# gereonsuch/gr-FDC

Hardware: AMD Instinct MI355X
Metric: complex Msamples/s in, 64k-FFT/256-ch overlap-save; achieved HBM GB/s vs peak (higher is better)
Workload: dtype f32

## Files before the change

gr-fdc_amd/csrc/fdc_block256.hip:

```cpp
#include "fdc_blockcommon.hpp"
#include "fdc_iq.hpp"

namespace fdc {

extern __shared__ __attribute__((aligned(16))) unsigned char fdc_smem_blk[];

typedef unsigned long long u8v __attribute__((ext_vector_type(8)));

template <int P, bool OFF, bool FWD, bool R4, class TO>
constexpr bool kBlkSpread = !OFF && !FWD && !(P == 8 && (R4 || !std::is_same<TO, float2>::value));

template <int P>
struct BlkGeom {
    static_assert(P == 2 || P == 4 || P == 8, "passes of 32 columns: N = 16384, 32768 or 65536");
    static constexpr int kN1 = 32 * P;
    static constexpr int kN = 256 * kN1;
    static constexpr int kJT = P == 8 ? 4 : 8;
    static constexpr int kJB = P == 8 ? 2 : P == 4 ? 4 : 8;
    static constexpr int kLd = P == 2 ? 32 * P + 2 : 32 * P + 6;
    static constexpr int kTripBytes = 16 * kJT * kLd * 8;
    static constexpr int kOffCt = kTripBytes > kStripsEnd ? kTripBytes : kStripsEnd;
    static constexpr int kOffWrow = P == 8 ? 136960 : kOffCt + 32 * P * 8;
    static constexpr bool kSplit = P > 2;
    static constexpr int kOffLT = kOffWrow + 16 * 18 * 8;
    static constexpr int kOffUR = kOffLT + 64 * 18 * 8;
    static constexpr int kOffB = kOffLT, kOffSA = kOffB + 32 * 18 * 8;
    static constexpr int kOffSoff = kSplit ? kOffUR + kN1 * 4 * 8 : kOffSA + 16 * P * 18 * 8;
    static constexpr int kOffCbl = kOffSoff + kN1 * 4;
    static constexpr int kLds = kOffCbl + (kSplit ? (P + 8) * 16 * 8 : 0);
    static constexpr int kOffWrowF = kLds;
    static constexpr int kLdsOff = kOffWrowF + 16 * 18 * 8;
    static_assert(kLdsOff <= 160 * 1024 && kLds <= 160 * 1024, "LDS budget");
    static_assert(kOffCt >= kStripsEnd && kOffCt + 32 * P * 8 <= kOffWrow, "stage-2 trip buffer and twiddles below the tables, tables above the strips");
    static_assert((16 * (kJB - 1) * kLd + 32 * (P - 1)) * 8 < 65536, "ds offsets of a base register");
};


template <int P, bool NT, bool OFF, bool FWD, bool R4 = false, bool HALF = false, class TI = float2, class TO = float2, bool SPREAD = false>
__global__ FDC_PLAIN_DS __launch_bounds__(512, (P == 2 && !OFF && !R4 && !FWD) ? 4 : 2) void k_blk256(const TI *__restrict__ in, size_t in_stride, TO *__restrict__ out,
                                                const float2 *__restrict__ tw256, const float2 *__restrict__ twq,
                                                const float2 *__restrict__ cbt, const float *__restrict__ shn,
                                                const long long *__restrict__ slot_off, long long out_base,
                                                long long nb_call, unsigned out_bytes, int nb, int hints,
                                                unsigned long long *__restrict__ dbg , int roff, long long first_block,
                                                float2 *__restrict__ fwd_scratch, const unsigned *__restrict__ keep,
                                                typename IqTail<TI, TO>::type gpow )
{
    typedef BlkGeom<P> GM;
    constexpr bool kIq = !std::is_same<TI, float2>::value, kOq = !std::is_same<TO, float2>::value;
    static_assert(!SPREAD || kBlkSpread<P, OFF, FWD, R4, TO>, "no spread form of this one");
    static_assert(!kIq || !FWD, "integer input: the channelizer forms (the forward transform takes widened input)");
    static_assert(!kOq || !FWD, "integer output: the channelizer forms");
    constexpr unsigned kEs = (unsigned)sizeof(TI);
    constexpr unsigned kOs = (unsigned)sizeof(TO);
    [[maybe_unused]] const float iq_scale = iq_tail_scale(gpow);
    [[maybe_unused]] const float oq_scale = oq_tail_scale(gpow);
    static_assert(!HALF || (!OFF && !FWD), "the half-slot form is a variant of the on-grid channelizer");
    constexpr int kN1 = GM::kN1, kLd = GM::kLd, kJT = GM::kJT, kJB = GM::kJB;
    float2 *scr = reinterpret_cast<float2 *>(fdc_smem_blk);
    float2 *wrow = reinterpret_cast<float2 *>(fdc_smem_blk + GM::kOffWrow);
    constexpr bool kSplit = GM::kSplit;
    float2 *LT = reinterpret_cast<float2 *>(fdc_smem_blk + GM::kOffLT);
    float2 *UR = reinterpret_cast<float2 *>(fdc_smem_blk + GM::kOffUR);
    float2 *CBL = reinterpret_cast<float2 *>(fdc_smem_blk + GM::kOffCbl);
    float2 *Bt = reinterpret_cast<float2 *>(fdc_smem_blk + GM::kOffB);
    float2 *SA = reinterpret_cast<float2 *>(fdc_smem_blk + GM::kOffSA);
    unsigned *soff = reinterpret_cast<unsigned *>(fdc_smem_blk + GM::kOffSoff);
    float2 *ctab = reinterpret_cast<float2 *>(fdc_smem_blk + GM::kOffCt);
    const int tid = threadIdx.x;
    const int w = tid >> 6, lane = tid & 63, col = lane & 3, b = lane >> 2, c5 = 4 * w + col;
    unsigned mqs[4] = {~0u, ~0u, ~0u, ~0u};
    if (FWD && keep) {
        const int wu = __builtin_amdgcn_readfirstlane(w) % P;
#pragma unroll
        for (int q = 0; q < 4; q++) mqs[q] = keep[wu * 4 + q];
    }

    const int grid = gridDim.x, first = xcd_first_block();
    if (first >= nb) return;

    constexpr unsigned inbytes = (unsigned)GM::kN * kEs;
    constexpr unsigned kRowGrp = (unsigned)kN1 * 16u * kEs;
    const unsigned voff = (unsigned)(b * kN1 + c5) * kEs;
    [[maybe_unused]] auto ld_in = [&](__amdgpu_buffer_rsrc_t r, unsigned soff, auto aux) __attribute__((always_inline)) -> cf {
        constexpr int kAux = decltype(aux)::value;
        if constexpr (sizeof(TI) == 4) return mk(__uint_as_float(__builtin_amdgcn_raw_buffer_load_b32(r, voff, soff, kAux)), 0.f);
        else return mk(__uint_as_float((unsigned)__builtin_amdgcn_raw_buffer_load_b16(r, voff, soff, kAux)), 0.f);
    };
    [[maybe_unused]] const __amdgpu_buffer_rsrc_t rcb = make_rsrc(cbt, (unsigned)kN1 * 16u * 8u);
    [[maybe_unused]] const unsigned voffc = (unsigned)(c5 * 16 + b) * 8u;
    cf LA[16], LB[16], cbA = mk(1.f, 0.f), cbB = cbA;
    {
        const __amdgpu_buffer_rsrc_t rin = make_rsrc(in + (size_t)first * in_stride, inbytes);
#pragma unroll
        for (int a = 0; a < 16; a++) {
            if constexpr (kIq) LA[a] = ld_in(rin, (unsigned)a * kRowGrp, std::integral_constant<int, 0>{});
            else LA[a] = bld2(rin, voff, (unsigned)a * kRowGrp);
        }
        if constexpr (!kSplit) cbA = bld2(rcb, voffc, 0);
    }
    float2 *wrowF = OFF ? reinterpret_cast<float2 *>(fdc_smem_blk + GM::kOffWrowF) : wrow;
    const int r16 = roff & 15;
    for (int i = tid; i < 256; i += 512) {
        const int ip = (i >> 4) * 18 + (((i & 15) - 1) & 15);
        wrow[ip] = tw256[((i >> 4) * (i & 15)) & 255];
        if (OFF)
            wrowF[ip] = tw256[((i >> 4) * ((((i & 15) - r16) & 15) + roff)) & 255];
    }
    for (int i = tid; i < kN1; i += 512) {
        const long long o = slot_off[i];
        soff[(i % P) * 32 + ((i / P) & 1) * 16 + rev16((i / P) >> 1)] = o >= 0 ? (unsigned)((o * nb_call + out_base) * kOs) : 0xFFFFFFFFu;
    }
    for (int i = tid; i < 32 * P; i += 512) ctab[i] = tw256[((i / P) * (i % P) * (8 / P)) & 255];
    if constexpr (kSplit) {
        for (int i = tid; i < 1024; i += 512) {
            const int ln = i >> 4, q = i & 15, qt = HALF ? q ^ 8 : q;
            const float2 t = twq[(ln & 3) * 16 + qt];
            const float s = shn[(ln >> 2) + 16 * qt];
            const float2 e = make_float2(t.x * s, t.y * s), c = cbt[(ln & 3) * 16 + (ln >> 2)];
            LT[ln * 18 + q] = make_float2(e.x * c.x - e.y * c.y, e.x * c.y + e.y * c.x);
        }
        for (int i = tid; i < kN1 * 4; i += 512) UR[i] = twq[(i >> 4) * 64 + (HALF ? (i & 15) ^ 8 : i & 15)];
        if (tid < (P + 8) * 16)
            CBL[tid] = cbt[(tid < P * 16 ? (tid >> 4) * 512 : ((tid >> 4) - P) * 64) + (tid & 15)];
    } else {
        Bt[(tid >> 4) * 18 + (tid & 15)] = twq[HALF ? tid ^ 8 : tid];
        for (int i = tid; i < 256 * P; i += 512) {
            const int ps = i >> 8, bb = (i >> 4) & 15, q = i & 15, qt = HALF ? q ^ 8 : q;
            const float2 t = twq[(size_t)(32 * ps) * 16 + qt];
            const float s = shn[bb + 16 * qt];
            SA[(ps * 16 + bb) * 18 + q] = make_float2(t.x * s, t.y * s);
        }
    }
    __syncthreads();

    float2 *const scrw = scr + w * kStripPts + lane;
    const float2 *const scrr = scr + w * kStripPts + col + 68 * b;
    const float2 *const wr = wrow + b * 18;
    const float2 *const wrf = wrowF + b * 18;
    const float2 *const tr0 = kSplit ? UR + w * 16 : Bt + c5 * 18;
    const float2 *const tr1 = kSplit ? LT + lane * 18 : SA + b * 18;
    const float2 *const cblr = CBL + b;
    const __amdgpu_buffer_rsrc_t rout = make_rsrc(out, out_bytes);
    constexpr bool kScr = FWD || R4;
    const __amdgpu_buffer_rsrc_t rscr = make_rsrc(kScr ? fwd_scratch + (size_t)blockIdx.x * 32768 : fwd_scratch, kScr ? 32768u * 8u : 0u);


    for (int m = first; m < nb; m += grid) {
        const int mnext = m + grid < nb ? m + grid : m;
        const float sgn = (OFF && !R4 && (roff & 1) && ((first_block + m) & 1)) ? -1.0f : 1.0f;
        cf phs = mk(1.f, 0.f);
        if constexpr (OFF && R4) {
            const int pc = (int)((((first_block + m) & 3) * (roff & 3)) & 3);
            phs = mk(pc == 0 ? 1.f : pc == 2 ? -1.f : 0.f, pc == 1 ? 1.f : pc == 3 ? -1.f : 0.f);
        }
        typedef unsigned long long gvec __attribute__((ext_vector_type(P)));
        gvec G[8];
#define FDC_GGET(j, ps) unpack_cf(G[j][ps])
#define FDC_GPUT(j, ps, val) G[j][ps] = pack_cf(val)
        auto one_pass = [&](const int ps, cf (&cur)[16], const cf cbc, cf (&L)[16], cf &cbn) __attribute__((always_inline)) {
            const cf cbl = kSplit ? cmul(ld2(&cblr[16 * ps]), ld2(&cblr[16 * (P + w)])) : cbc;
            const cf cb = (OFF && R4) ? cmul(cbl, phs) : OFF ? cbl * sgn : cbl;
            const int pn = ps < P - 1 ? ps + 1 : 0;
            const int mb = ps < P - 1 ? m : mnext;
            const __amdgpu_buffer_rsrc_t rin = make_rsrc(in + (size_t)mb * in_stride + 32 * pn, inbytes);
            if constexpr (!SPREAD) {
                if constexpr (kIq) {
                    if (hints & 2) {
#pragma unroll
                        for (int a = 0; a < 16; a++) L[a] = ld_in(rin, (unsigned)a * kRowGrp, std::integral_constant<int, 2>{});
                    } else {
#pragma unroll
                        for (int a = 0; a < 16; a++) L[a] = ld_in(rin, (unsigned)a * kRowGrp, std::integral_constant<int, 0>{});
                    }
                } else if (hints & 2) {
#pragma unroll
                    for (int a = 0; a < 16; a++) L[a] = bld2_nt(rin, voff, (unsigned)a * kRowGrp);
                } else {
#pragma unroll
                    for (int a = 0; a < 16; a++) L[a] = bld2(rin, voff, (unsigned)a * kRowGrp);
                }
                if constexpr (!kSplit) cbn = bld2(rcb, voffc, (unsigned)pn * 4096u);
            }
            auto ld_rows = [&](auto group) __attribute__((always_inline)) {
                constexpr int g = decltype(group)::value;
                if constexpr (SPREAD) {
                    __builtin_amdgcn_sched_barrier(0);
#pragma unroll
                    for (int a = 4 * g; a < 4 * g + 4; a++) {
                        if constexpr (kIq) L[a] = ld_in(rin, (unsigned)a * kRowGrp, std::integral_constant<int, 0>{});
                        else L[a] = bld2(rin, voff, (unsigned)a * kRowGrp);
                    }
                    if constexpr (!kSplit && g == 3) cbn = bld2(rcb, voffc, (unsigned)pn * 4096u);
                }
            };
            const float2 *const r0 = tr0 + (kSplit ? 128 * ps : 0), *const r1 = tr1 + (kSplit ? 0 : 288 * ps);
            if constexpr (kIq) {
#pragma unroll
                for (int a = 0; a < 16; a++) cur[a] = iq_widen_bits(TI{}, __float_as_uint(cur[a].x), iq_scale);
            }
            dft16<false>(cur);
            ld_rows(std::integral_constant<int, 0>{});
            cf tw[16];
            ld_row_sh<OFF>(tw, wrf);
            if constexpr (OFF) {
#pragma unroll
                for (int p = 0; p < 16; p++) st2(&scrw[68 * ((p - r16) & 15)], cmul(cur[rev16(p)], tw[p]));
            } else {
                st2(&scrw[0], cur[rev16(0)]);
#pragma unroll
                for (int p = 1; p < 16; p++) st2(&scrw[68 * p], cmul(cur[rev16(p)], tw[p]));
            }
            __builtin_amdgcn_wave_barrier();
            cf v[16];
            strip_get(v, scrr);
            if constexpr (FWD) {
                dft16<false>(v);
#pragma unroll
                for (int i = 0; i < 8; i++) {
                    const float4 t0 = ld4(&r0[2 * i]), t1 = ld4(&r1[2 * i]);
                    const cf y0 = cmul(cmul(cmul(v[rev16(2 * i)], mk(t0.x, t0.y)), mk(t1.x, t1.y)), cb);
                    const cf y1 = cmul(cmul(cmul(v[rev16(2 * i + 1)], mk(t0.z, t0.w)), mk(t1.z, t1.w)), cb);
                    if (i < 4) { FDC_GPUT(2 * i, ps, y0); FDC_GPUT(2 * i + 1, ps, y1); }
                    else {
                        bst2(rscr, (unsigned)tid * 8u + (unsigned)(2 * i - 8) * 4096u, (unsigned)ps * 32768u, y0);
                        bst2(rscr, (unsigned)tid * 8u + (unsigned)(2 * i - 7) * 4096u, (unsigned)ps * 32768u, y1);
                    }
                }
            } else {
                dft16<false>(v);
                ld_rows(std::integral_constant<int, 1>{});
                cf u[16];
                {
#pragma unroll
                    for (int i = 0; i < 8; i++) {
                        const float4 t0 = ld4(&r0[2 * i]), t1 = ld4(&r1[2 * i]);
                        u[HALF ? 2 * i : (2 * i) ^ 8] = cmul(cmul(v[rev16(2 * i)], mk(t0.x, t0.y)), mk(t1.x, t1.y));
                        u[HALF ? 2 * i + 1 : (2 * i + 1) ^ 8] = cmul(cmul(v[rev16(2 * i + 1)], mk(t0.z, t0.w)), mk(t1.z, t1.w));
                    }
                }
                dft16<true>(u);
                ld_rows(std::integral_constant<int, 2>{});
                ld_row_sh<false>(tw, wr);
                u[rev16(0)] = cmul(u[rev16(0)], cb);
#pragma unroll
                for (int p = 1; p < 16; p++) u[rev16(p)] = cmul(cmulc(u[rev16(p)], tw[p]), cb);
                strip_trip(u, scrw, scrr);
                ld_rows(std::integral_constant<int, 3>{});
                dft16<true>(u);
                if constexpr (SPREAD) __builtin_amdgcn_sched_barrier(0);
#pragma unroll
                for (int j = 0; j < 8; j++) FDC_GPUT(j, ps, u[rev16(8 + j)]);
                if constexpr (SPREAD) __builtin_amdgcn_sched_barrier(0);
                if constexpr (R4) {
#pragma unroll
                    for (int j = 0; j < 4; j++) bst2(rscr, (unsigned)tid * 8u + (unsigned)j * 4096u, (unsigned)ps * 16384u, u[rev16(4 + j)]);
                }
            }
        };
        if constexpr (OFF && P == 8) {
#pragma nounroll
            for (int ps = 0; ps < P; ps++) {
                cf cur[16];
#pragma unroll
                for (int a = 0; a < 16; a++) cur[a] = LA[a];
                one_pass(ps, cur, cbA, LA, cbA);
            }
        } else {
#pragma nounroll
            for (int pp = 0; pp < P; pp += 2) {
                one_pass(pp, LA, cbA, LB, cbB);
                one_pass(pp + 1, LB, cbB, LA, cbA);
            }
        }
        auto stage2 = [&](auto get, const int rowbase, auto njc) __attribute__((always_inline)) {
            constexpr int kNJ = decltype(njc)::value;
            constexpr int kNTrip = (kNJ + kJT - 1) / kJT;
            __syncthreads();
            int t2 = tid;
            asm volatile("" : "+v"(t2));
            const int lane2 = t2 & 63, w2 = __builtin_amdgcn_readfirstlane(t2 >> 6), b_2 = lane2 >> 2, c5_2 = 4 * w2 + (lane2 & 3);
            const int klo2 = w2 % P, rh2 = w2 / P;
            float2 *const gw0 = scr + b_2 * kLd + c5_2;
            int rowjb = 16 * kJB * kLd;
            asm volatile("" : "+v"(rowjb));
            float2 *const gw1 = gw0 + rowjb;
            const float2 *const gr = scr + (64 * rh2 + lane2) * kLd + 32 * klo2;
            const uint4 *const sow = reinterpret_cast<const uint4 *>(soff + 32 * klo2);
#pragma unroll
            for (int tr = 0; tr < kNTrip; tr++) {
                const int ja = kNJ - kJT * tr < kJT ? kNJ - kJT * tr : kJT;
                cf ct[P];
                {
                    const float2 *ctr = reinterpret_cast<const float2 *>(fdc_smem_blk + GM::kOffCt) + c5_2 * P;
#pragma unroll
                    for (int i = 0; i < P / 2; i++) {
                        const float4 t = ld4(&ctr[2 * i]);
                        ct[2 * i] = mk(t.x, t.y); ct[2 * i + 1] = mk(t.z, t.w);
                    }
                }
                cf src[kJT][P];
#pragma unroll
                for (int jj = 0; jj < kJT; jj++)
#pragma unroll
                    for (int ps = 0; ps < P; ps++) if (jj < ja) src[jj][ps] = get(kJT * tr + jj, ps);
#pragma unroll
                for (int jj = 0; jj < kJT; jj++) {
                    if (jj >= ja) continue;
                    cf a[P];
#pragma unroll
                    for (int ps = 0; ps < P; ps++) a[ps] = src[jj][ps];
                    pass_dft<P>(a);
                    float2 *const gw = (jj < kJB ? gw0 : gw1) + (jj % kJB) * 16 * kLd;
                    st2(&gw[0], a[0]);
#pragma unroll
                    for (int k = 1; k < P; k++) st2(&gw[32 * k], cmul(a[pass_idx<P>(k)], ct[k]));
                }
                __builtin_amdgcn_sched_barrier(0);
                __syncthreads();
                const bool reads = P == 8 || 4 * rh2 < ja;
                cf v[32];
                if (reads) {
#pragma unroll
                    for (int i = 0; i < 16; i++) {
                        const float4 t = ld4(&gr[2 * i]);
                        v[2 * i] = mk(t.x, t.y); v[2 * i + 1] = mk(t.z, t.w);
                    }
                }
                __syncthreads();
                __builtin_amdgcn_sched_barrier(0);
                if (reads) {
                    dft32<false>(v);
                    const int trow0 = 16 * kJT * tr + 64 * rh2, trow = trow0 + lane2;
                    const unsigned rb = (unsigned)(m * (FWD ? GM::kN : (R4 ? 192 : 128)) + rowbase + trow) * kOs;
                    unsigned mq = FWD ? mqs[((rowbase + trow0) >> 6) & 3] : ~0u;
                    if constexpr (FWD) asm volatile("" : "+s"(mq));
#pragma unroll
                    for (int q = 0; q < 8; q++) {
                        const uint4 t = sow[q];
                        const unsigned so[4] = {t.x, t.y, t.z, t.w};
#pragma unroll
                        for (int e = 0; e < 4; e++) {
                            const unsigned o = FWD ? (so[e] | (((mq >> (4 * q + e)) & 1u) - 1u)) : so[e];
                            if constexpr (kOq) {
                                const unsigned u = oq_bits(TO{}, v[4 * q + e], oq_scale);
                                if constexpr (kOs == 4) __builtin_amdgcn_raw_buffer_store_b32(u, rout, (o == 0xFFFFFFFFu ? 0xFFFFFFF0u : o + rb), 0, NT ? 2 : 0);
                                else __builtin_amdgcn_raw_buffer_store_b16((unsigned short)u, rout, (o == 0xFFFFFFFFu ? 0xFFFFFFF0u : o + rb), 0, NT ? 2 : 0);
                            } else
                                bst2t<NT>(rout, (o == 0xFFFFFFFFu ? 0xFFFFFFF0u : o + rb), v[4 * q + e]);
                        }
                    }
                    if constexpr (FWD) {
                        if (gpow) {
                            float t16[16];
#pragma unroll
                            for (int i = 0; i < 16; i++) {
                                const float s0 = __builtin_fmaf(v[i].y, v[i].y, v[i].x * v[i].x);
                                const float s1 = __builtin_fmaf(v[i + 16].y, v[i + 16].y, v[i + 16].x * v[i + 16].x);
                                asm("s_nop 1\n\tv_add_f32_dpp %0, %1, %1 row_ror:8 row_mask:0xf bank_mask:0x3\n\t"
                                    "v_add_f32_dpp %0, %2, %2 row_ror:8 row_mask:0xf bank_mask:0xc" : "=&v"(t16[i]) : "v"(s0), "v"(s1));
                            }
                            float t8[8];
#pragma unroll
                            for (int i = 0; i < 8; i++)
                                asm("s_nop 1\n\tv_add_f32_dpp %0, %1, %1 row_shl:4 row_mask:0xf bank_mask:0x5\n\t"
                                    "v_add_f32_dpp %0, %2, %2 row_shr:4 row_mask:0xf bank_mask:0xa" : "=&v"(t8[i]) : "v"(t16[i]), "v"(t16[i + 8]));
                            const bool b1 = (lane2 & 2) != 0, b0 = (lane2 & 1) != 0;
                            float t4[4], t2[2];
#pragma unroll
                            for (int i = 0; i < 4; i++) {
                                const float keepv = b1 ? t8[i + 4] : t8[i], send = b1 ? t8[i] : t8[i + 4];
                                t4[i] = keepv + __builtin_bit_cast(float, __builtin_amdgcn_update_dpp(0, __builtin_bit_cast(int, send), 0x4E , 0xF, 0xF, false));
                            }
#pragma unroll
                            for (int i = 0; i < 2; i++) {
                                const float keepv = b0 ? t4[i + 2] : t4[i], send = b0 ? t4[i] : t4[i + 2];
                                t2[i] = keepv + __builtin_bit_cast(float, __builtin_amdgcn_update_dpp(0, __builtin_bit_cast(int, send), 0xB1 , 0xF, 0xF, false));
                            }
                            const int i16 = lane2 & 15, rho = lane2 >> 4, gsrc = 2 * (i16 & 1);
                            const int a0 = (16 * gsrc + 4 * rho + (i16 >> 2)) * 4, a1 = a0 + 64;
                            const int z0 = __builtin_bit_cast(int, t2[0]), z1 = __builtin_bit_cast(int, t2[1]);
                            const int f0a = __builtin_amdgcn_ds_bpermute(a0, z0), f0b = __builtin_amdgcn_ds_bpermute(a0, z1);
                            const int f1a = __builtin_amdgcn_ds_bpermute(a1, z0), f1b = __builtin_amdgcn_ds_bpermute(a1, z1);
                            const bool odd = (i16 & 2) != 0;
                            float2 pr;
                            pr.x = __builtin_bit_cast(float, odd ? f0b : f0a);
                            pr.y = __builtin_bit_cast(float, odd ? f1b : f1a);
                            const int reg = 8 * rho + (i16 >> 1), slot = klo2 + P * ((reg >> 4) + 2 * (4 * (reg & 3) + ((reg & 15) >> 2)));
                            *reinterpret_cast<float2 *>(gpow + (size_t)m * (GM::kN / 16) + 16 * slot + (rowbase + trow0) / 16 + gsrc) = pr;
                        }
                    }
                }
                __builtin_amdgcn_sched_barrier(0);
            }
        };
        stage2([&](int j, int ps) { return FDC_GGET(j, ps); }, R4 ? 64 : 0, std::integral_constant<int, 8>{});
        if constexpr (FWD) {
            asm volatile("s_waitcnt vmcnt(0)" ::: "memory");
            stage2([&](int j, int ps) { return bld2_sc1(rscr, (unsigned)tid * 8u + (unsigned)(j * 4096 + ps * 32768), 0u); }, 128,
                   std::integral_constant<int, 8>{});
        }
        if constexpr (R4) {
            asm volatile("s_waitcnt vmcnt(0)" ::: "memory");
            stage2([&](int j, int ps) { return bld2_sc1(rscr, (unsigned)tid * 8u + (unsigned)(j * 4096 + ps * 16384), 0u); }, 0,
                   std::integral_constant<int, 4>{});
        }
    }
}

template <int P, bool NT, bool OFF, bool FWD, bool R4, bool HALF, class TI, class TO, bool SPREAD>
constexpr bool blk256_form()
{
    constexpr bool kIq = !std::is_same<TI, float2>::value, kOq = !std::is_same<TO, float2>::value;
    constexpr bool kOqR4Narrowed = P == 8 && R4 && !kIq && kOq;
    return (!kOq || NT) && !kOqR4Narrowed && !(HALF && OFF) && (!FWD || !(kIq || kOq || OFF || R4 || HALF)) && (!SPREAD || kBlkSpread<P, OFF, FWD, R4, TO>);
}

template <class F>
static void for_blk256_forms(int p, int nt, int off, int fwd, int r4, int half, int ifmt, int ofmt, int spread, F &&f)
{
    auto form = [&](auto P, auto NT, auto OFF, auto FWD, auto R4, auto HALF, auto ti, auto to) {
        using TI = decltype(ti);
        using TO = decltype(to);
        constexpr bool kNt = NT() != 0, kOff = OFF() != 0, kFwd = FWD() != 0, kR4 = R4() != 0, kHalf = HALF() != 0;
        constexpr int kLds = kOff ? BlkGeom<P()>::kLdsOff : BlkGeom<P()>::kLds;
        if constexpr (blk256_form<P(), kNt, kOff, kFwd, kR4, kHalf, TI, TO, false>()) {
            constexpr bool kTwin = blk256_form<P(), kNt, kOff, kFwd, kR4, kHalf, TI, TO, true>();
            if (spread != 1 || !kTwin) f(k_blk256<P(), kNt, kOff, kFwd, kR4, kHalf, TI, TO, false>, kLds, ti, to);
            if constexpr (kTwin)
                if (spread != 0) f(k_blk256<P(), kNt, kOff, kFwd, kR4, kHalf, TI, TO, true>, kLds, ti, to);
        }
    };
    for_values<2, 4, 8>(p, [&](auto P) { for_values<1, 0>(nt, [&](auto NT) { for_values<0, 1>(off, [&](auto OFF) { for_values<0, 1>(fwd, [&](auto FWD) {
        for_values<0, 1>(r4, [&](auto R4) { for_values<0, 1>(half, [&](auto HALF) {
            for_samples(ifmt, [&](auto ti) { for_samples(ofmt, [&](auto to) { form(P, NT, OFF, FWD, R4, HALF, ti, to); }); });
        }); });
    }); }); }); });
}

hipError_t init_block_kernels()
{
    hipError_t e = hipSuccess;
    for_blk256_forms(kEvery, kEvery, kEvery, kEvery, kEvery, kEvery, kEvery, kEvery, kEvery, [&](auto k, int lds, auto, auto) {
        if (e == hipSuccess) e = set_block_lds(reinterpret_cast<const void *>(k), lds);
    });
    return e;
}

bool poly_block_supports(int N) { return N == 16384 || N == 32768 || N == 65536; }

hipError_t launch_poly_block(const BlockLaunch &b)
{
    if (b.nb_chunk <= 0) return hipSuccess;
    const bool r4 = b.R == 4, halfslot = b.half();
    if (b.L != 256 || b.r < 0 || b.r >= 256 || !poly_block_supports(b.N) || (b.R != 2 && !r4) || (r4 && !b.scratch)) return hipErrorInvalidValue;
    if (b.ifmt == kEvery || b.ofmt == kEvery) return hipErrorInvalidValue;
    const int grid = b.grid(b.N == 16384 && b.R == 2 && (!b.r || halfslot) ? 2 : 1);
    hipError_t e = hipErrorInvalidValue;
    for_blk256_forms(b.N / 8192, b.hints & 1, !halfslot && b.r, 0, r4, halfslot, b.ifmt, b.ofmt, !(b.hints & 2), [&](auto k, int lds, auto ti, auto to) {
        using TI = decltype(ti);
        using TO = decltype(to);
        hipExtLaunchKernelGGL(k, dim3((unsigned)grid), dim3(512), lds, b.s, b.ev_start, b.ev_stop, 0u, static_cast<const TI *>(b.in), b.in_stride,
                              static_cast<TO *>(b.out), b.tw256, b.twq, b.cbt, b.shn, b.slot_off, (long long)b.mbase * (r4 ? 192 : 128), (long long)b.nb_call,
                              b.out_bytes, b.nb_chunk, b.hints, (unsigned long long *)nullptr, halfslot ? 0 : b.r, b.first_block,
                              r4 ? b.scratch : (float2 *)nullptr, (const unsigned *)nullptr, iq_tail<TI, TO>(nullptr, b.iscale, b.oscale));
        e = hipGetLastError();
    });
    return e;
}

hipError_t launch_block_fft(int N, const float2 *in, size_t in_stride, float2 *out, int nitems, const float2 *tw256,
                            const float2 *twq, const float2 *cbt0, const float *shn1, const long long *slot_off,
                            float2 *scratch , int ncu, int hints, hipStream_t s, hipEvent_t *ev,
                            const unsigned *keep, float *gpow )
{
    if (!poly_block_supports(N)) return hipErrorInvalidValue;
    const int per = (int)(((size_t)1 << 28) / (size_t)N);
    for (int m0 = 0; m0 < nitems; m0 += per) {
        const int nb = nitems - m0 < per ? nitems - m0 : per;
        int grid = ncu > 0 ? ncu : 256;
        if (grid > nb) grid = nb;
        hipEvent_t e0 = ev && m0 == 0 ? ev[0] : nullptr, e2 = ev && m0 + nb >= nitems ? ev[1] : nullptr;
        hipError_t e = hipErrorInvalidValue;
        for_blk256_forms(N / 8192, hints & 1, 0, 1, 0, 0, kIqFloat, kIqFloat, 0, [&](auto k, int lds, auto ti, auto to) {
            if constexpr (std::is_same<decltype(ti), float2>::value && std::is_same<decltype(to), float2>::value) {
                hipExtLaunchKernelGGL(k, dim3((unsigned)grid), dim3(512), lds, s, e0, e2, 0u, in + (size_t)m0 * in_stride, in_stride, out + (size_t)m0 * (size_t)N,
                                      tw256, twq, cbt0, shn1, slot_off, 0ll, 1ll, (unsigned)((size_t)nb * (size_t)N * 8), nb, hints,
                                      (unsigned long long *)nullptr, 0, 0ll, scratch, keep, gpow ? gpow + (size_t)m0 * (size_t)(N / 16) : (float *)nullptr);
                e = hipGetLastError();
            }
        });
        if (e != hipSuccess) return e;
    }
    if (ev) { hipError_t e = hipEventRecord(ev[2], s); if (e != hipSuccess) return e; }
    return hipGetLastError();
}

}
```

Measured before the change: 218,600.

## Read per-wave twiddle row through scalar loads and precompute full cb table

```diff
diff --git a/gr-fdc_amd/csrc/fdc_block256.hip b/gr-fdc_amd/csrc/fdc_block256.hip
--- a/gr-fdc_amd/csrc/fdc_block256.hip
+++ b/gr-fdc_amd/csrc/fdc_block256.hip
@@ -7,12 +7,27 @@
 
 typedef unsigned long long u8v __attribute__((ext_vector_type(8)));
 
+typedef unsigned int u32x8 __attribute__((ext_vector_type(8)));
+typedef __attribute__((address_space(4))) u32x8 srow_piece;
+__device__ __forceinline__ cf cmul_s(cf a, cf b)
+{
+    cf r;
+    asm("v_pk_mul_f32 %0, %1, %2 op_sel_hi:[0,1]\n\t"
+        "v_pk_fma_f32 %0, %1, %2, %0 op_sel:[1,1,0] op_sel_hi:[1,0,1] neg_lo:[0,1,0]"
+        : "=&v"(r) : "v"(a), "s"(b));
+    return r;
+}
+
 template <int P, bool OFF, bool FWD, bool R4, class TO>
 constexpr bool kBlkSpread = !OFF && !FWD && !(P == 8 && (R4 || !std::is_same<TO, float2>::value));
 
-template <int P>
+template <int P, bool OFF, bool FWD, bool R4>
+constexpr bool kBlkSrow = P == 8 && !OFF && !FWD && !R4;
+
+template <int P, bool SROW = false>
 struct BlkGeom {
     static_assert(P == 2 || P == 4 || P == 8, "passes of 32 columns: N = 16384, 32768 or 65536");
+    static_assert(!SROW || P > 2, "the scalar wave row replaces UR, which P = 2 does not have");
     static constexpr int kN1 = 32 * P;
     static constexpr int kN = 256 * kN1;
     static constexpr int kJT = P == 8 ? 4 : 8;
@@ -25,14 +40,16 @@
     static constexpr int kOffLT = kOffWrow + 16 * 18 * 8;
     static constexpr int kOffUR = kOffLT + 64 * 18 * 8;
     static constexpr int kOffB = kOffLT, kOffSA = kOffB + 32 * 18 * 8;
-    static constexpr int kOffSoff = kSplit ? kOffUR + kN1 * 4 * 8 : kOffSA + 16 * P * 18 * 8;
+    static constexpr int kOffSoff = kSplit ? kOffUR + (SROW ? 0 : kN1 * 4 * 8) : kOffSA + 16 * P * 18 * 8;
     static constexpr int kOffCbl = kOffSoff + kN1 * 4;
-    static constexpr int kLds = kOffCbl + (kSplit ? (P + 8) * 16 * 8 : 0);
+    static constexpr int kCblRows = SROW ? kN1 / 4 : P + 8;
+    static constexpr int kLds = kOffCbl + (kSplit ? kCblRows * 16 * 8 : 0);
     static constexpr int kOffWrowF = kLds;
     static constexpr int kLdsOff = kOffWrowF + 16 * 18 * 8;
     static_assert(kLdsOff <= 160 * 1024 && kLds <= 160 * 1024, "LDS budget");
     static_assert(kOffCt >= kStripsEnd && kOffCt + 32 * P * 8 <= kOffWrow, "stage-2 trip buffer and twiddles below the tables, tables above the strips");
     static_assert((16 * (kJB - 1) * kLd + 32 * (P - 1)) * 8 < 65536, "ds offsets of a base register");
+    static_assert(!SROW || kCblRows * 16 * 8 == kN1 * 4 * 8, "the whole cb table takes what UR had: the total shrinks by the two-factor table");
 };
 
 
@@ -46,7 +63,8 @@
                                                 float2 *__restrict__ fwd_scratch, const unsigned *__restrict__ keep,
                                                 typename IqTail<TI, TO>::type gpow )
 {
-    typedef BlkGeom<P> GM;
+    constexpr bool kSrow = kBlkSrow<P, OFF, FWD, R4>;
+    typedef BlkGeom<P, kSrow> GM;
     constexpr bool kIq = !std::is_same<TI, float2>::value, kOq = !std::is_same<TO, float2>::value;
     static_assert(!SPREAD || kBlkSpread<P, OFF, FWD, R4, TO>, "no spread form of this one");
     static_assert(!kIq || !FWD, "integer input: the channelizer forms (the forward transform takes widened input)");
@@ -120,9 +138,13 @@
             const float2 e = make_float2(t.x * s, t.y * s), c = cbt[(ln & 3) * 16 + (ln >> 2)];
             LT[ln * 18 + q] = make_float2(e.x * c.x - e.y * c.y, e.x * c.y + e.y * c.x);
         }
-        for (int i = tid; i < kN1 * 4; i += 512) UR[i] = twq[(i >> 4) * 64 + (HALF ? (i & 15) ^ 8 : i & 15)];
-        if (tid < (P + 8) * 16)
-            CBL[tid] = cbt[(tid < P * 16 ? (tid >> 4) * 512 : ((tid >> 4) - P) * 64) + (tid & 15)];
+        if constexpr (kSrow) {
+            for (int i = tid; i < kN1 * 4; i += 512) CBL[i] = cbt[(i >> 4) * 64 + (i & 15)];
+        } else {
+            for (int i = tid; i < kN1 * 4; i += 512) UR[i] = twq[(i >> 4) * 64 + (HALF ? (i & 15) ^ 8 : i & 15)];
+            if (tid < (P + 8) * 16)
+                CBL[tid] = cbt[(tid < P * 16 ? (tid >> 4) * 512 : ((tid >> 4) - P) * 64) + (tid & 15)];
+        }
     } else {
         Bt[(tid >> 4) * 18 + (tid & 15)] = twq[HALF ? tid ^ 8 : tid];
         for (int i = tid; i < 256 * P; i += 512) {
@@ -140,7 +162,8 @@
     const float2 *const wrf = wrowF + b * 18;
     const float2 *const tr0 = kSplit ? UR + w * 16 : Bt + c5 * 18;
     const float2 *const tr1 = kSplit ? LT + lane * 18 : SA + b * 18;
-    const float2 *const cblr = CBL + b;
+    const float2 *const cblr = CBL + b + (kSrow ? 16 * w : 0);
+    [[maybe_unused]] const srow_piece *const srow = (const srow_piece *)(unsigned long long)(twq + (kSrow ? 64 * __builtin_amdgcn_readfirstlane(w) : 0));
     const __amdgpu_buffer_rsrc_t rout = make_rsrc(out, out_bytes);
     constexpr bool kScr = FWD || R4;
     const __amdgpu_buffer_rsrc_t rscr = make_rsrc(kScr ? fwd_scratch + (size_t)blockIdx.x * 32768 : fwd_scratch, kScr ? 32768u * 8u : 0u);
@@ -159,7 +182,7 @@
 #define FDC_GGET(j, ps) unpack_cf(G[j][ps])
 #define FDC_GPUT(j, ps, val) G[j][ps] = pack_cf(val)
         auto one_pass = [&](const int ps, cf (&cur)[16], const cf cbc, cf (&L)[16], cf &cbn) __attribute__((always_inline)) {
-            const cf cbl = kSplit ? cmul(ld2(&cblr[16 * ps]), ld2(&cblr[16 * (P + w)])) : cbc;
+            const cf cbl = kSrow ? ld2(&cblr[128 * ps]) : kSplit ? cmul(ld2(&cblr[16 * ps]), ld2(&cblr[16 * (P + w)])) : cbc;
             const cf cb = (OFF && R4) ? cmul(cbl, phs) : OFF ? cbl * sgn : cbl;
             const int pn = ps < P - 1 ? ps + 1 : 0;
             const int mb = ps < P - 1 ? m : mnext;
@@ -199,8 +222,14 @@
 #pragma unroll
                 for (int a = 0; a < 16; a++) cur[a] = iq_widen_bits(TI{}, __float_as_uint(cur[a].x), iq_scale);
             }
+            [[maybe_unused]] auto ld_piece = [&](int k) __attribute__((always_inline)) -> u32x8 {
+                __builtin_amdgcn_sched_barrier(0);
+                return srow[128 * ps + (HALF ? k ^ 2 : k)];
+            };
+            [[maybe_unused]] u32x8 pc[2];
             dft16<false>(cur);
             ld_rows(std::integral_constant<int, 0>{});
+            if constexpr (kSrow) { pc[0] = ld_piece(0); pc[1] = ld_piece(1); }
             cf tw[16];
             ld_row_sh<OFF>(tw, wrf);
             if constexpr (OFF) {
@@ -231,7 +260,24 @@
                 dft16<false>(v);
                 ld_rows(std::integral_constant<int, 1>{});
                 cf u[16];
-                {
+                if constexpr (kSrow) {
+#pragma unroll
+                    for (int h = 0; h < 2; h++) {
+                        cf t[8];
+#pragma unroll
+                        for (int j = 0; j < 8; j++) {
+                            const u32x8 pj = pc[j >> 2];
+                            t[j] = cmul_s(v[rev16(8 * h + j)], mk(__uint_as_float(pj[2 * (j & 3)]), __uint_as_float(pj[2 * (j & 3) + 1])));
+                        }
+                        if (h == 0) { pc[0] = ld_piece(2); pc[1] = ld_piece(3); }
+#pragma unroll
+                        for (int i = 0; i < 4; i++) {
+                            const float4 t1 = ld4(&r1[8 * h + 2 * i]);
+                            u[HALF ? 8 * h + 2 * i : (8 * h + 2 * i) ^ 8] = cmul(t[2 * i], mk(t1.x, t1.y));
+                            u[HALF ? 8 * h + 2 * i + 1 : (8 * h + 2 * i + 1) ^ 8] = cmul(t[2 * i + 1], mk(t1.z, t1.w));
+                        }
+                    }
+                } else {
 #pragma unroll
                     for (int i = 0; i < 8; i++) {
                         const float4 t0 = ld4(&r0[2 * i]), t1 = ld4(&r1[2 * i]);
@@ -423,7 +469,8 @@
         using TI = decltype(ti);
         using TO = decltype(to);
         constexpr bool kNt = NT() != 0, kOff = OFF() != 0, kFwd = FWD() != 0, kR4 = R4() != 0, kHalf = HALF() != 0;
-        constexpr int kLds = kOff ? BlkGeom<P()>::kLdsOff : BlkGeom<P()>::kLds;
+        constexpr bool kSrow = kBlkSrow<P(), kOff, kFwd, kR4>;
+        constexpr int kLds = kOff ? BlkGeom<P()>::kLdsOff : BlkGeom<P(), kSrow>::kLds;
         if constexpr (blk256_form<P(), kNt, kOff, kFwd, kR4, kHalf, TI, TO, false>()) {
             constexpr bool kTwin = blk256_form<P(), kNt, kOff, kFwd, kR4, kHalf, TI, TO, true>();
             if (spread != 1 || !kTwin) f(k_blk256<P(), kNt, kOff, kFwd, kR4, kHalf, TI, TO, false>, kLds, ti, to);
```

Result: faster. 223,400 (median of 6 runs) (+2.2%).
